# sleveque/control

Measured on AMD Instinct MI355X. Metric: Krylov iterations/s (preconditioned GMRES(10), all-at-once heat-control KKT), higher is better.
Workload: dtype f64; 1 GPU; 2-D heat control, 256^2 P1, n_t=64, beta=0.0001, T=2, BE, mode G; unknowns=8454272, krylov=gmres, left preconditioning, restart 10, classical Gram-Schmidt, parallelism=time-block rows over 1 GPU(s), transport=none, sweep_tiles=boxes from the dof coordinates (kkt_set_tile_coordinates)

## Files before the change

control_amd/csrc/tile_kernels.hip:

```cpp
#include "kernels.hpp"

#include <hip/hip_runtime.h>

#include "epilogue.hpp"

#include <algorithm>
#include <type_traits>

namespace kkt {

#define KKT_GLOBAL __attribute__((address_space(1)))
typedef KKT_GLOBAL const double *gcd_p;
typedef KKT_GLOBAL double *gd_p;
typedef KKT_GLOBAL const int32_t *gci_p;
typedef KKT_GLOBAL const uint16_t *gcu16_p;
typedef KKT_GLOBAL const uint8_t *gcb_p;
typedef KKT_GLOBAL unsigned long long *gu64_p;
typedef unsigned int u32x4 __attribute__((ext_vector_type(4)));

constexpr unsigned TILE_SPIN_LIMIT = 1u << 21;

__device__ __forceinline__ void lds_barrier() {
    asm volatile("s_waitcnt lgkmcnt(0)\n\ts_barrier" ::: "memory");
}

__device__ __forceinline__ void publish(const __amdgpu_buffer_rsrc_t rs, int grow, double v,
                                        unsigned tag) {
    const unsigned long long bits = (unsigned long long)__double_as_longlong(v);
    const u32x4 g = {(unsigned)bits, tag, (unsigned)(bits >> 32), tag};
    __builtin_amdgcn_raw_buffer_store_b128(g, rs, grow * 16, 0, 16 );
}

struct LevEarly {
    const double *vals, *dinv, *bin, *upd0;
    int32_t n_upd, prev_in_lds;
};
__device__ __forceinline__ LevEarly read_early(const TileLevel *p) {
    LevEarly f;
    f.vals = p->vals;
    f.dinv = p->dinv;
    f.bin = p->bin;
    f.upd0 = p->upd_vals[0];
    f.n_upd = p->n_upd;
    f.prev_in_lds = p->prev_in_lds;
    return f;
}

template <typename P>
__device__ __forceinline__ P opaque_ptr(P p) {
    unsigned long long u = (unsigned long long)p;
    asm volatile("" : "+v"(u));
    return (P)u;
}
__device__ __forceinline__ unsigned opaque(unsigned x) {
    asm volatile("" : "+v"(x));
    return x;
}

__device__ __forceinline__ unsigned uniform(unsigned x) { return __builtin_amdgcn_readfirstlane(x); }
template <typename P>
__device__ __forceinline__ P uniform_ptr(P p) {
    const unsigned long long u = (unsigned long long)p;
    return (P)(((unsigned long long)uniform((unsigned)(u >> 32)) << 32) | uniform((unsigned)u));
}
constexpr int TILE_NO_POLL = 0x7ffffff0;

template <int W, int RPT, int TMAX, bool UPD, int HPT_ = RPT + 1, bool COARSE = false>
__global__ __launch_bounds__(TMAX) void pc_tile_sweep(
    const TileArgs A, const TileLevel *__restrict__ levels, const int32_t *__restrict__ n_all,
    const int32_t *__restrict__ grow_all, const uint16_t *__restrict__ lcol_all,
    const int32_t *__restrict__ gpos_all, const uint8_t *__restrict__ rowmask_) {
    constexpr int HPT = HPT_;
    extern __shared__ double X[];
    __shared__ int sn[TILE_DEPTH_MAX + 1];
    __shared__ int sdead;
    __shared__ unsigned long long sstat[8];
    const int T = blockDim.x, tid = threadIdx.x, tile = blockIdx.x;
    const int nkp = A.nk_pad, depth = A.depth, its = A.its;
    const int32_t *nt = n_all + (size_t)tile * (TILE_DEPTH_MAX + 1);
    const int n0 = nt[0], nk = nt[depth], nk1 = nt[depth - 1];
    if (tid <= TILE_DEPTH_MAX) sn[tid] = nt[tid];
    if (tid < 8) sstat[tid] = 0ull;
    if (tid == 0) {
        sdead = 0;
        X[nkp - 1] = 0.0;
        X[2 * (size_t)nkp - 1] = 0.0;
    }
    __shared__ int s_bail;
    if (tid == 0) {
        typedef KKT_GLOBAL unsigned long long *gu64a_p;
        const gu64a_p ctr = (gu64a_p)(A.err + 2), bail = (gu64a_p)(A.err + 4);
        const unsigned long long nt_ = gridDim.x;
        const bool skip = A.debug_drop < 0 && tile == 0;
        unsigned long long old = 0ull;
        if (!skip) old = __hip_atomic_fetch_add(ctr, 1ull, __ATOMIC_RELAXED, __HIP_MEMORY_SCOPE_AGENT);
        else old = __hip_atomic_load(ctr, __ATOMIC_RELAXED, __HIP_MEMORY_SCOPE_AGENT);
        const unsigned long long target = (old / nt_ + 1ull) * nt_;
        int bad = 0;
        unsigned long long seen = old;
        for (int spin = 0; spin < 4096; ++spin) {
            seen = __hip_atomic_load(ctr, __ATOMIC_RELAXED, __HIP_MEMORY_SCOPE_AGENT);
            if (seen >= target) break;
            if (__hip_atomic_load(bail, __ATOMIC_RELAXED, __HIP_MEMORY_SCOPE_AGENT) == target) break;
            __builtin_amdgcn_s_sleep(8);
        }
        if (seen < target) {
            __hip_atomic_store(bail, target, __ATOMIC_RELAXED, __HIP_MEMORY_SCOPE_AGENT);
            bad = 1;
        } else if (__hip_atomic_load(bail, __ATOMIC_RELAXED, __HIP_MEMORY_SCOPE_AGENT) == target) {
            bad = 1;
        }
        if (bad) {
            atomicOr(A.err, 8u);
            if (atomicCAS(A.err + 1, 0u, 1u) == 0u) {
                A.err[17] = (unsigned)(seen - (target - nt_));
                A.err[18] = (unsigned)nt_;
            }
        }
        s_bail = bad;
    }
    __syncthreads();
    if (s_bail) return;

    const gci_p grow = (gci_p)grow_all + (size_t)tile * nkp;
    const gcb_p rowmask = (gcb_p)rowmask_;

    constexpr bool PACK = W > 9;
    constexpr int CH = PACK ? 5 : W;
    constexpr int WP = (W + 1) / 2;
    constexpr int CW = PACK ? WP : W, GW = PACK ? 1 : W;
    unsigned cpk[RPT][CW];
    int gpr[RPT][GW];
    int gr[RPT];
    bool msk[RPT];
    const gcu16_p lcol = (gcu16_p)lcol_all + (size_t)tile * RPT * W * T + tid;
    const gci_p gpos = (gci_p)gpos_all + (size_t)tile * RPT * W * T + tid;
    const gci_p gpos_base = gpos;
#pragma unroll
    for (int sl = 0; sl < RPT; ++sl) {
        const int r = sl * T + tid;
        if constexpr (PACK) {
#pragma unroll
            for (int k = 0; k < W; k += 2) {
                const unsigned lo = lcol[(size_t)(sl * W + k) * T];
                const unsigned hi = k + 1 < W ? lcol[(size_t)(sl * W + k + 1) * T] : 0u;
                cpk[sl][k / 2] = lo | (hi << 16);
            }
            gpr[sl][0] = 0;
        } else {
#pragma unroll
            for (int k = 0; k < W; ++k) {
                cpk[sl][k] = lcol[(size_t)(sl * W + k) * T];
                gpr[sl][k] = gpos[(size_t)(sl * W + k) * T];
            }
        }
        gr[sl] = r < nk1 ? grow[r] : -1;
        msk[sl] = gr[sl] >= 0 && rowmask != nullptr && rowmask[gr[sl]] != 0;
    }
    constexpr bool OPQ = PACK && TMAX > 512;
    constexpr bool TIGHT = COARSE;
    auto idx = [](const int i) { return TIGHT ? (int)opaque((unsigned)i) : i; };
    auto at = [&](const gcd_p p, const int i, const bool live) -> double {
        return live ? p[idx(i)] : 0.0;
    };
#define KKT_CPK(sl, j) (OPQ ? opaque(cpk[sl][j]) : cpk[sl][j])
#define KKT_COL(sl, k)                                                                       \
    (int)(PACK ? (((k) & 1) ? (KKT_CPK(sl, PACK ? (k) / 2 : 0) >> 16)                         \
                            : (KKT_CPK(sl, PACK ? (k) / 2 : 0) & 0xffffu))                    \
               : cpk[sl][PACK ? 0 : (k)])
#define KKT_GP(sl, k) (PACK ? gpos[(size_t)((sl) * W + (k)) * T] : gpr[sl][PACK ? 0 : (k)])
    int hl[HPT], hg[HPT];
#pragma unroll
    for (int h = 0; h < HPT; ++h) {
        const int l = n0 + h * T + tid;
        hl[h] = l < nk ? l : -1;
        hg[h] = l < nk ? grow[l] : 0;
    }

    double *scoef = X + 2 * (size_t)nkp;
    double *dump = scoef + 3 * (size_t)(COARSE ? (its > 0 ? its : 1) : (its > 1 ? its - 1 : 1));
    double *SL = dump + 1, *RC = nullptr, *EC = nullptr;
    int c_nc = 0, c_jmax = 0, c_pstride = 0, c_nslots = 0, c_nj = 0, c_slot0 = 0;
    bool c_rings = false;
    int c_njp = 0, c_jx = 0;
    unsigned cepoch = A.cepoch0;
    void *cg0 = nullptr, *cg1 = nullptr, *eg0 = nullptr, *eg1 = nullptr;
    int cg_bytes = 0, eg_bytes = 0;
    if constexpr (COARSE) {
        const TileCoarseDev *cd = A.coarse;
        cg0 = uniform_ptr((void *)cd->cg[0]);
        cg1 = uniform_ptr((void *)cd->cg[1]);
        eg0 = uniform_ptr((void *)cd->eg[0]);
        eg1 = uniform_ptr((void *)cd->eg[1]);
        cg_bytes = (int)uniform(cd->cg_bytes);
        eg_bytes = (int)uniform(cd->eg_bytes);
        c_nc = cd->nc;
        c_jmax = cd->jmax;
        c_pstride = cd->pstride;
        c_nslots = cd->nslots;
        c_nj = cd->nj[tile];
        c_slot0 = cd->slot0[tile];
        c_rings = cd->ring_prolong != 0;
        c_njp = c_rings ? cd->njx[tile] : c_nj;
        c_jx = c_rings ? cd->jxmax : c_jmax;
        RC = SL + c_nslots;
        EC = RC + c_nc;
    }
    double *RWc = nullptr, *PWc = nullptr;
    int *CSLc = nullptr, *CIPc = nullptr, *RIPc = nullptr, *JGc = nullptr;
    int *PIPc = nullptr;
    uint16_t *RROWc = nullptr, *PKc = nullptr;
    gci_p c_pip = nullptr;
    bool c_cached = true;
    int c_re0 = 0, c_pq0 = 0;
    double *EINVc = nullptr;
    bool c_einv_cache = false;
    const void *einv_key = nullptr;
    const int c_nown = COARSE ? (c_nc > tile ? (c_nc - tile + (int)gridDim.x - 1) / (int)gridDim.x : 0) : 0;
    int c_lo0 = 0, c_hi0 = 0, c_ew = 0;
    if constexpr (COARSE) {
        const TileCoarseDev *cd = A.coarse;
        c_ew = cd->ew;
        if ((int)(threadIdx.x >> 6) < c_nown) {
            const int j0 = tile + (int)(threadIdx.x >> 6) * (int)gridDim.x;
            c_lo0 = cd->e_lo[j0];
            c_hi0 = cd->e_hi[j0];
        }
        c_cached = cd->cache_lists != 0;
        const int nrm = c_cached ? cd->nr_max : 0;
        const int npm = c_rings ? cd->np_max : nrm;
        RWc = EC + c_jx;
        PWc = RWc + nrm;
        CSLc = reinterpret_cast<int *>(PWc + npm);
        CIPc = CSLc + c_nslots;
        RIPc = CIPc + (c_nc + 1);
        JGc = RIPc + (c_jmax + 1);
        PIPc = JGc + c_jx;
        RROWc = reinterpret_cast<uint16_t *>(PIPc + (c_rings ? nkp + 1 : 0));
        PKc = RROWc + nrm;
        c_einv_cache = cd->cache_einv != 0;
        EINVc = reinterpret_cast<double *>(
            (reinterpret_cast<uintptr_t>(PKc + npm) + 7) & ~(uintptr_t)7);
        const gci_p rip = (gci_p)cd->r_ip + (size_t)tile * c_jmax;
        const gci_p pip = (gci_p)cd->p_ip + (size_t)tile * c_pstride;
        const int re0 = (int)uniform((unsigned)rip[0]), re1 = (int)uniform((unsigned)rip[c_nj]);
        const int pq0 = (int)uniform((unsigned)pip[0]);
        const int pq1 = (int)uniform((unsigned)pip[c_rings ? nk : nt[0]]);
        c_re0 = re0;
        c_pq0 = pq0;
        const gcu16_p rrow = (gcu16_p)cd->r_row, pk = (gcu16_p)cd->p_k;
        const gcd_p rw = (gcd_p)cd->r_w, pw = (gcd_p)cd->p_w;
        if (c_cached) {
            for (int i = tid; i < re1 - re0; i += T) {
                RWc[i] = rw[re0 + i];
                RROWc[i] = rrow[re0 + i];
            }
            for (int i = tid; i < pq1 - pq0; i += T) {
                PWc[i] = pw[pq0 + i];
                PKc[i] = pk[pq0 + i];
            }
        }
        const gci_p cslot = (gci_p)cd->c_slot, cip = (gci_p)cd->c_ip;
        for (int i = tid; i < c_nslots; i += T) CSLc[i] = cslot[i];
        for (int i = tid; i <= c_nc; i += T) CIPc[i] = cip[i];
        const gci_p jg = (gci_p)cd->jglob + (size_t)tile * cd->jxmax;
        for (int i = tid; i <= c_nj; i += T) RIPc[i] = rip[i] - re0;
        for (int i = tid; i < c_njp; i += T) JGc[i] = jg[i];
        if (c_rings)
            for (int i = tid; i <= nk; i += T) PIPc[i] = pip[i] - pq0;
        c_pip = pip;
        __syncthreads();
    }
    const void *coef_key = nullptr;
    int cur = 0;
    unsigned epoch = A.epoch0;
    bool dead = false;
    const void *vals_key = nullptr;
    double v[RPT][W];

    unsigned long long *stat = reinterpret_cast<unsigned long long *>(A.err + 64) + (size_t)tile * 8;
    const bool stamps = A.stamps != 0;
    unsigned long long t_mark = stamps ? wall_clock64() : 0ull;
    auto lap = [&](int slot, unsigned long long count) {
        if (!stamps) return;
        const unsigned long long now = wall_clock64();
#ifndef KKT_XSTAMPS
        if (tid == 0) {
            sstat[slot] += now - t_mark;
            sstat[slot + 3] += count;
        }
#else
        if (tid == 0 && slot == 0) sstat[3] += count;
#endif
        t_mark = now;
    };

    static_assert(sizeof(TileLevel) == 128, "two scalar-cache lines per level");
    LevEarly Nf{};
    bool nf_valid = false;
    const TileLevel *nf_want = nullptr;
    auto handoff = [&](const bool both, const bool early = false) {
        lap(1, 0);
        if (nf_want != nullptr) {
            Nf = read_early(nf_want);
            nf_want = nullptr;
            nf_valid = true;
        }
        ++epoch;
        double *Xc = X + cur * nkp, *Xo = X + (cur ^ 1) * nkp;
        const __amdgpu_buffer_rsrc_t rn = __builtin_amdgcn_make_buffer_rsrc(
            uniform_ptr((void *)A.gnew[epoch & 1]), 0, (int)A.granule_bytes, 0x00020000);
        const __amdgpu_buffer_rsrc_t ro = __builtin_amdgcn_make_buffer_rsrc(
            uniform_ptr((void *)A.gold[epoch & 1]), 0, (int)A.granule_bytes, 0x00020000);
#pragma unroll
        for (int sl = 0; sl < RPT; ++sl) {
            const int r = sl * T + tid;
            if (r < n0 && !(tile == 0 && A.debug_drop > 0 && (int)(epoch - A.epoch0) == A.debug_drop)) {
                if (!early) publish(rn, gr[sl], Xc[r], epoch);
                if (both && depth > 1) publish(ro, gr[sl], Xo[r], epoch);
            }
        }
        bool want_o[HPT], need_n[HPT], need_o[HPT];
#pragma unroll
        for (int h = 0; h < HPT; ++h) {
            want_o[h] = both && hl[h] >= 0 && hl[h] < nk1;
            need_n[h] = hl[h] >= 0;
            need_o[h] = want_o[h];
        }
        auto value = [](const u32x4 g) {
            return __longlong_as_double((long long)((unsigned long long)g.x | ((unsigned long long)g.z << 32)));
        };
        for (int i = 0; i < A.poll_delay; ++i) __builtin_amdgcn_s_sleep(1);
        unsigned spins = 0;
        while (true) {
            asm volatile("" ::: "memory");
            bool ok = true;
            u32x4 tn[HPT], to[HPT];
#pragma unroll
            for (int h = 0; h < HPT; ++h) {
                tn[h] = __builtin_amdgcn_raw_buffer_load_b128(
                    rn, need_n[h] ? hg[h] * 16 : TILE_NO_POLL, 0, 16 );
                to[h] = __builtin_amdgcn_raw_buffer_load_b128(
                    ro, need_o[h] ? hg[h] * 16 : TILE_NO_POLL, 0, 16 );
            }
            __builtin_amdgcn_sched_barrier(0);
            unsigned seen[HPT][4];
#pragma unroll
            for (int h = 0; h < HPT; ++h) {
                seen[h][0] = need_n[h] ? tn[h].y : (hl[h] >= 0 ? epoch : 0u);
                seen[h][1] = need_n[h] ? tn[h].w : (hl[h] >= 0 ? epoch : 0u);
                seen[h][2] = need_o[h] ? to[h].y : (want_o[h] ? epoch : 0u);
                seen[h][3] = need_o[h] ? to[h].w : (want_o[h] ? epoch : 0u);
                const bool hit_n = need_n[h] && tn[h].y == epoch && tn[h].w == epoch;
                const bool hit_o = need_o[h] && to[h].y == epoch && to[h].w == epoch;
                if (hit_n) Xc[hl[h]] = value(tn[h]);
                if (hit_o) Xo[hl[h]] = value(to[h]);
                need_n[h] = need_n[h] && !hit_n;
                need_o[h] = need_o[h] && !hit_o;
                ok &= !need_n[h] && !need_o[h];
            }
            if (ok || dead) break;
            if (++spins >= TILE_SPIN_LIMIT) {
                dead = true;
                sdead = 1;
                atomicOr(A.err, 4u);
                if (atomicCAS(A.err + 1, 0u, 1u) == 0u) {
#pragma unroll
                    for (int h = 0; h < HPT; ++h)
                        if (need_n[h] || need_o[h]) {
                            A.err[8] = (unsigned)tile;
                            A.err[9] = epoch;
                            A.err[10] = (unsigned)hl[h];
                            A.err[11] = (unsigned)hg[h];
                            A.err[12] = seen[h][0];
                            A.err[13] = seen[h][1];
                            A.err[14] = seen[h][2];
                            A.err[15] = seen[h][3];
                            A.err[16] = both ? 1u : 0u;
                        }
                }
                break;
            }
            __builtin_amdgcn_s_sleep(1);
        }
        lds_barrier();
        dead = sdead != 0;
#ifndef KKT_XSTAMPS
        if (stamps && tid == 0) sstat[6] += spins;
#endif
        lap(0, 1);
    };

    double dinv[RPT], b[RPT];
    auto load_vals = [&](const double *ptr, const bool update_matrix) {
        vals_key = uniform_ptr((const void *)ptr);
        const gcd_p vp = (gcd_p)ptr;
        if constexpr (PACK) {
            const gci_p gpos = opaque_ptr(gpos_base);
            constexpr int G = RPT * W > 30 ? 1 : RPT;
#pragma unroll
            for (int s0 = 0; s0 < RPT; s0 += G) {
                int gp[G][W];
#pragma unroll
                for (int q = 0; q < G; ++q)
#pragma unroll
                    for (int k = 0; k < W; ++k) gp[q][k] = KKT_GP(s0 + q, k);
                __builtin_amdgcn_sched_barrier(0);
#pragma unroll
                for (int q = 0; q < G; ++q)
#pragma unroll
                    for (int k = 0; k < W; ++k)
                        v[s0 + q][k] = at(vp, gp[q][k],
                                          gp[q][k] >= 0 && (!update_matrix || gr[s0 + q] >= 0));
                __builtin_amdgcn_sched_barrier(0);
            }
        } else {
#pragma unroll
            for (int sl = 0; sl < RPT; ++sl)
#pragma unroll
                for (int k = 0; k < W; ++k) {
                    const int gp = idx(KKT_GP(sl, k));
                    v[sl][k] = at(vp, gp, gp >= 0 && (!update_matrix || idx(gr[sl]) >= 0));
                }
        }
    };
    auto load_db = [&](const LevEarly &L) {
        const gcd_p dp = (gcd_p)L.dinv, bp = (gcd_p)L.bin;
#pragma unroll
        for (int sl = 0; sl < RPT; ++sl) {
            dinv[sl] = at(dp, gr[sl], idx(gr[sl]) >= 0);
            b[sl] = at(bp, gr[sl], idx(gr[sl]) >= 0);
        }
    };
    auto load_level = [&](const LevEarly &L) {
        if (uniform_ptr((const void *)L.vals) != vals_key) load_vals(L.vals, false);
        load_db(L);
    };
    constexpr bool SEQ = (PACK || COARSE) && UPD;
    bool v_is_u = false;
    if (A.nlevels > 0) {
        const LevEarly L0 = read_early(&levels[0]);
        if (SEQ && L0.n_upd > 0) {
            load_vals(L0.upd0, true);
            load_db(L0);
            v_is_u = true;
        } else {
            load_level(L0);
        }
    }

    constexpr bool PRE = UPD && !COARSE && W * RPT <= 14 && TMAX <= 512;
    constexpr bool PRE_U = UPD && !COARSE && !PRE && W * RPT <= 7;
    constexpr int PR = PRE ? RPT : 1, PW = PRE ? W : 1;
    constexpr int UR = (PRE || PRE_U) ? RPT : 1, UW = (PRE || PRE_U) ? W : 1;
    double vn[PR][PW], un[UR][UW], dn[PR], bn[PR];
    bool pre_v = false, pre_u = false, pre_issued = false, un_loaded = false;
    auto load_un = [&](const LevEarly &N) {
        if constexpr (PRE || PRE_U) {
            pre_u = N.n_upd > 0;
            if (pre_u) {
                const gcd_p up = (gcd_p)N.upd0;
#pragma unroll
                for (int sl = 0; sl < RPT; ++sl)
#pragma unroll
                    for (int k = 0; k < W; ++k) {
                        const int gp = KKT_GP(sl, k);
                        un[sl][k] = (gr[sl] >= 0 && gp >= 0) ? up[gp] : 0.0;
                    }
            }
            un_loaded = true;
        }
    };
    auto prefetch_level = [&](const LevEarly &N) {
        if constexpr (PRE) {
            pre_issued = true;
            pre_v = uniform_ptr((const void *)N.vals) != vals_key;
            if (pre_v) {
                const gcd_p vp = (gcd_p)N.vals;
#pragma unroll
                for (int sl = 0; sl < RPT; ++sl)
#pragma unroll
                    for (int k = 0; k < W; ++k) {
                        const int gp = KKT_GP(sl, k);
                        vn[sl][k] = gp >= 0 ? vp[gp] : 0.0;
                    }
            }
            load_un(N);
            const gcd_p dp = (gcd_p)N.dinv, bp = (gcd_p)N.bin;
#pragma unroll
            for (int sl = 0; sl < RPT; ++sl) {
                dn[sl] = gr[sl] >= 0 ? dp[gr[sl]] : 0.0;
                bn[sl] = gr[sl] >= 0 ? bp[gr[sl]] : 0.0;
            }
        }
    };
    auto adopt_level = [&](const LevEarly &N) {
        if constexpr (PRE) {
            if (pre_v) {
                vals_key = uniform_ptr((const void *)N.vals);
#pragma unroll
                for (int sl = 0; sl < RPT; ++sl)
#pragma unroll
                    for (int k = 0; k < W; ++k) v[sl][k] = vn[sl][k];
            }
#pragma unroll
            for (int sl = 0; sl < RPT; ++sl) {
                dinv[sl] = dn[sl];
                b[sl] = bn[sl];
            }
        }
    };

    for (int lev = 0; lev < A.nlevels; ++lev) {
        const TileLevel &L = levels[lev];
        nf_valid = false;
        nf_want = lev + 1 < A.nlevels ? &levels[lev + 1] : nullptr;
        const bool have_u = (PRE || PRE_U) && un_loaded && pre_u;
        const bool use_v = SEQ && v_is_u;
        pre_issued = false;
        un_loaded = false;
        v_is_u = false;
        const double *einv_lev = nullptr;
        if constexpr (COARSE) {
            typedef const double *einv_entry;
            typedef __attribute__((address_space(4))) const einv_entry *einv_table_p;
            einv_lev = ((einv_table_p)(uintptr_t)A.einv)[lev];
        }
        if (uniform_ptr((const void *)L.coef) != coef_key) {
            coef_key = uniform_ptr((const void *)L.coef);
            const gcd_p cp = (gcd_p)(const double *)L.coef;
            __syncthreads();
            for (int i = idx(tid); i < 3 * (COARSE ? its : its - 1); i += T) scoef[i] = cp[i];
        }
#pragma unroll
        for (int sl = 0; sl < RPT; ++sl) {
            if constexpr (!(SEQ && COARSE)) {
#pragma unroll
                for (int k = 0; k < W; ++k) asm volatile("" : "+v"(v[sl][k]));
            }
            asm volatile("" : "+v"(dinv[sl]));
            asm volatile("" : "+v"(b[sl]));
        }
        if (!COARSE && stamps && tid == 0) sstat[7] += wall_clock64() - t_mark;
        const double post1 = L.post1, post2 = L.post2;
        int cr;
        {
            double *Xc = X + cur * nkp, *Xo = X + (cur ^ 1) * nkp;
            if (UPD && L.n_upd > 0) {
                if (!L.prev_in_lds) {
                    const gcd_p xp = (gcd_p)L.x_prev;
                    for (int l = idx(tid); l < nk; l += T) Xc[l] = xp[grow[l]];
                    lds_barrier();
                }
                double acc[RPT];
#pragma unroll
                for (int sl = 0; sl < RPT; ++sl) acc[sl] = 0.0;
                if constexpr (PRE || PRE_U) {
                    if (have_u) {
                        double xu[UR][UW];
#pragma unroll
                        for (int sl = 0; sl < RPT; ++sl)
#pragma unroll
                            for (int k = 0; k < W; ++k) xu[sl][k] = Xc[KKT_COL(sl, k)];
                        __builtin_amdgcn_sched_barrier(0);
#pragma unroll
                        for (int k = 0; k < W; ++k)
#pragma unroll
                            for (int sl = 0; sl < RPT; ++sl)
                                acc[sl] = __builtin_fma(un[sl][k], xu[sl][k], acc[sl]);
                    }
                }
                if constexpr (SEQ) {
                    if (use_v) {
#pragma unroll
                        for (int sl = 0; sl < RPT; ++sl) {
                            if (sl * T + (tid & ~63) >= nk1) continue;
#pragma unroll
                            for (int k0 = 0; k0 < W; k0 += CH) {
                                double xv[CH];
#pragma unroll
                                for (int k = 0; k < CH; ++k)
                                    if (k0 + k < W) xv[k] = Xc[KKT_COL(sl, k0 + k)];
#pragma unroll
                                for (int k = 0; k < CH; ++k)
                                    if (k0 + k < W)
                                        acc[sl] = __builtin_fma(v[sl][k0 + k], xv[k], acc[sl]);
                                __builtin_amdgcn_sched_barrier(0);
                            }
                        }
                    }
                }
                if constexpr (!(PACK && SEQ))
                for (int t = (have_u || use_v) ? 1 : 0; t < L.n_upd; ++t) {
                    const gcd_p up = (gcd_p)L.upd_vals[t];
#pragma unroll
                    for (int sl = 0; sl < RPT; ++sl) {
                        if (sl * T + (tid & ~63) >= nk1) continue;
#pragma unroll
                        for (int k0 = 0; k0 < W; k0 += CH) {
                            int gp[CH];
                            double vu[CH];
#pragma unroll
                            for (int k = 0; k < CH; ++k)
                                if (k0 + k < W) gp[k] = idx(KKT_GP(sl, k0 + k));
#pragma unroll
                            for (int k = 0; k < CH; ++k)
                                if (k0 + k < W)
                                    vu[k] = at(up, gp[k], idx(gr[sl]) >= 0 && gp[k] >= 0);
#pragma unroll
                            for (int k = 0; k < CH; ++k)
                                if (k0 + k < W)
                                    acc[sl] = __builtin_fma(vu[k], Xc[KKT_COL(sl, k0 + k)], acc[sl]);
                            if constexpr (PACK) __builtin_amdgcn_sched_barrier(0);
                        }
                    }
                }
                if constexpr (SEQ && COARSE) {
                    if (uniform_ptr((const void *)L.vals) != vals_key) load_vals(L.vals, false);
                }
                const gd_p bo = (gd_p)L.bout;
#pragma unroll
                for (int sl = 0; sl < RPT; ++sl) {
                    const int r = sl * T + tid;
                    const double out =
                        msk[sl] ? 0.0 : epi_lin(L.ca, acc[sl], true, L.cy, b[sl], false, 0.0, 0.0);
                    const double out2 = epi_first(L.p1_scale, dinv[sl], out);
                    b[sl] = out;
                    if (r < nk1) Xo[r] = out2;
                    if (r < n0 && bo != nullptr) bo[idx(gr[sl])] = out;
                }
                if constexpr (SEQ && !COARSE) {
                    if (uniform_ptr((const void *)L.vals) != vals_key) load_vals(L.vals, false);
                }
            } else {
                const bool last = its == 1;
                const double q1 = last ? post1 : 1.0, q2 = last ? post2 : 1.0;
#pragma unroll
                for (int sl = 0; sl < RPT; ++sl) {
                    const int r = sl * T + tid;
                    double out = 0.0;
                    if (!msk[sl])
                        out = epi_cheb(false, 0.0, 0.0, false, 0.0, 0.0, L.p1_scale, dinv[sl], b[sl],
                                       0.0, q1, q2);
                    if (r < nk1) Xo[r] = out;
                }
            }
            cr = depth - 1;
            lds_barrier();
            cur ^= 1;
        }
        const bool has_next = lev + 1 < A.nlevels;
        if (PRE && has_next && its - 1 <= cr) {
            Nf = read_early(&levels[lev + 1]);
            nf_want = nullptr;
            nf_valid = true;
            prefetch_level(Nf);
        }
#pragma unroll
        for (int sl = 0; sl < RPT; ++sl) {
            if constexpr (SEQ && !COARSE) {
#pragma unroll
                for (int k = 0; k < W; ++k) asm volatile("" : "+v"(v[sl][k]));
            }
            asm volatile("" : "+v"(dinv[sl]));
            asm volatile("" : "+v"(b[sl]));
        }
        lap(2, 1);
        if constexpr (COARSE) {
            auto cstep = [&](const int mode, const int nv, const double cf1, const double cf2,
                             const double cf3, const bool has_old, const double q1,
                             const double q2) {
                double *Xc = X + cur * nkp, *Xo = X + (cur ^ 1) * nkp;
#pragma unroll
                for (int sl = 0; sl < RPT; ++sl) {
                    if (sl * T + (tid & ~63) >= nv) continue;
                    const int r = sl * T + tid;
                    double acc = 0.0;
#pragma unroll
                    for (int k0 = 0; k0 < W; k0 += CH) {
                        double xv[CH];
#pragma unroll
                        for (int k = 0; k < CH; ++k)
                            if (k0 + k < W) xv[k] = Xc[KKT_COL(sl, k0 + k)];
#pragma unroll
                        for (int k = 0; k < CH; ++k)
                            if (k0 + k < W) acc = __builtin_fma(v[sl][k0 + k], xv[k], acc);
                        if constexpr (PACK) __builtin_amdgcn_sched_barrier(0);
                    }
                    if (r < nv) {
                        double out = 0.0;
                        if (!msk[sl]) {
                            if (mode == 0) {
                                out = epi_cheb(has_old, cf1, Xo[r], true, cf2, Xc[r], cf3, dinv[sl],
                                               b[sl], acc, q1, q2);
                            } else {
                                out = b[sl] - acc;
                            }
                        }
                        Xo[r] = out;
                    }
                }
            };
            const TileCoarseDev *cd = A.coarse;
            const gcd_p einv = (gcd_p)einv_lev;
            const int wave = tid >> 6, lane = tid & 63, nwaves = T >> 6;
            for (int cyc = 0; cyc < A.cycles; ++cyc) {
                if (cyc == 0) {
                    double *Xo = X + (cur ^ 1) * nkp;
#pragma unroll
                    for (int sl = 0; sl < RPT; ++sl) {
                        const int r = sl * T + tid;
                        if (r < n0) Xo[r] = b[sl];
                    }
                } else {
                    if (cr == 0 || (c_rings && cr < depth)) {
                        handoff(false);
                        cr = depth;
                    }
                    cstep(1, n0, 0.0, 0.0, 0.0, false, 1.0, 1.0);
                }
                lds_barrier();
                lap(1, cyc == 0 ? 0 : 1);
#ifdef KKT_XSTAMPS
                unsigned long long xs_t = wall_clock64();
                auto xs = [&](int slot) {
                    const unsigned long long n_ = wall_clock64();
                    if (tid == 0) sstat[slot] += n_ - xs_t;
                    xs_t = n_;
                };
#define KKT_XS(slot) xs(slot)
#else
#define KKT_XS(slot)
#endif
                ++cepoch;
                {
                    int pe0[RPT], pe1[RPT];
                    if (!c_rings) {
#pragma unroll
                        for (int sl = 0; sl < RPT; ++sl) {
                            const int r = sl * T + tid;
                            pe0[sl] = r < n0 ? c_pip[r] - c_pq0 : 0;
                            pe1[sl] = r < n0 ? c_pip[r + 1] - c_pq0 : 0;
                        }
                    }
                    const double *Rb = X + (cur ^ 1) * nkp;
                    const __amdgpu_buffer_rsrc_t rc_ = __builtin_amdgcn_make_buffer_rsrc(
                        (cepoch & 1) ? cg1 : cg0, 0, cg_bytes, 0x00020000);
                    for (int k = wave; k < c_nj; k += nwaves) {
                        const int e0 = RIPc[k], e1 = RIPc[k + 1];
                        double a = 0.0;
                        if (c_cached) {
                            for (int e = e0 + lane; e < e1; e += 64)
                                a = __builtin_fma(RWc[e], Rb[RROWc[e]], a);
                        } else {
                            const gcu16_p rrow = (gcu16_p)cd->r_row + c_re0;
                            const gcd_p rw = (gcd_p)cd->r_w + c_re0;
                            for (int e = e0 + lane; e < e1; e += 64)
                                a = __builtin_fma(rw[e], Rb[rrow[e]], a);
                        }
#pragma unroll
                        for (int o = 32; o > 0; o >>= 1) a += __shfl_xor(a, o, 64);
                        if (lane == 0) publish(rc_, c_slot0 + k, a, cepoch);
                    }
                    constexpr int CSL = 4;
                    KKT_XS(0);
                    for (int i = 0; i < A.poll_delay; ++i) __builtin_amdgcn_s_sleep(1);
                    for (int base = 0; base < c_nslots; base += CSL * T) {
                        bool need[CSL];
#pragma unroll
                        for (int q = 0; q < CSL; ++q) need[q] = base + q * T + tid < c_nslots;
                        const bool live0 = need[0];
                        unsigned spins = 0;
                        while (true) {
                            asm volatile("" ::: "memory");
                            bool ok = true;
                            u32x4 t[CSL];
#pragma unroll
                            for (int q = 0; q < CSL; ++q)
                                t[q] = __builtin_amdgcn_raw_buffer_load_b128(
                                    rc_, need[q] ? (base + q * T + tid) * 16 : TILE_NO_POLL, 0, 16);
                            __builtin_amdgcn_sched_barrier(0);
                            const unsigned seen_y = need[0] ? t[0].y : (live0 ? cepoch : 0u);
                            const unsigned seen_w = need[0] ? t[0].w : (live0 ? cepoch : 0u);
#pragma unroll
                            for (int q = 0; q < CSL; ++q) {
                                const bool hit = need[q] && t[q].y == cepoch && t[q].w == cepoch;
                                if (hit)
                                    SL[base + q * T + tid] = __longlong_as_double((long long)(
                                        (unsigned long long)t[q].x | ((unsigned long long)t[q].z << 32)));
                                need[q] = need[q] && !hit;
                                ok &= !need[q];
                            }
                            if (ok || dead) break;
                            if (++spins >= TILE_SPIN_LIMIT) {
                                dead = true;
                                sdead = 1;
                                atomicOr(A.err, 4u);
                                if (atomicCAS(A.err + 1, 0u, 1u) == 0u) {
                                    A.err[8] = (unsigned)tile;
                                    A.err[9] = cepoch;
                                    A.err[10] = 0xffffu;
                                    A.err[11] = (unsigned)(base + tid);
                                    A.err[12] = seen_y;
                                    A.err[13] = seen_w;
                                    A.err[16] = 2u;
                                }
                                break;
                            }
                            __builtin_amdgcn_s_sleep(1);
                        }
                    }
                    KKT_XS(1);
                    lds_barrier();
                    KKT_XS(2);
                    dead = sdead != 0;
                    for (int j = tid; j < c_nc; j += T) {
                        double a = 0.0;
                        for (int q = CIPc[j]; q < CIPc[j + 1]; ++q) a += SL[CSLc[q]];
                        RC[j] = a;
                    }
                    lds_barrier();
                    KKT_XS(4);
                    const __amdgpu_buffer_rsrc_t re_ = __builtin_amdgcn_make_buffer_rsrc(
                        (cepoch & 1) ? eg1 : eg0, 0, eg_bytes, 0x00020000);
                    const int ntl = (int)gridDim.x;
                    const gci_p elo = (gci_p)cd->e_lo, ehi = (gci_p)cd->e_hi;
                    if (c_einv_cache && uniform_ptr((const void *)einv) != einv_key) {
                        for (int i = wave; i < c_nown; i += nwaves) {
                            const int j = tile + i * ntl;
                            const int lo = i == wave ? c_lo0 : elo[j], hi = i == wave ? c_hi0 : ehi[j];
                            const gcd_p row = einv + (size_t)j * c_nc;
                            for (int q = lo + lane; q < hi; q += 64)
                                EINVc[(size_t)i * c_ew + (q - lo)] = row[q];
                        }
                        einv_key = uniform_ptr((const void *)einv);
                    }
                    for (int i = wave; i < c_nown; i += nwaves) {
                        double a = 0.0;
                        const int j = tile + i * ntl;
                        const int lo = i == wave ? c_lo0 : elo[j], hi = i == wave ? c_hi0 : ehi[j];
                        if (c_einv_cache) {
                            const double *row = EINVc + (size_t)i * c_ew;
                            for (int q = lo + lane; q < hi; q += 64)
                                a = __builtin_fma(row[q - lo], RC[q], a);
                        } else {
                            const gcd_p row = einv + (size_t)j * c_nc;
                            constexpr int EU = 8;
                            for (int q0 = lo + lane; q0 < hi; q0 += 64 * EU) {
                                double rv[EU];
#pragma unroll
                                for (int u = 0; u < EU; ++u) {
                                    const int q = q0 + 64 * u;
                                    rv[u] = q < hi ? row[q] : 0.0;
                                }
#pragma unroll
                                for (int u = 0; u < EU; ++u) {
                                    const int q = q0 + 64 * u;
                                    if (q < hi) a = __builtin_fma(rv[u], RC[q], a);
                                }
                            }
                        }
#pragma unroll
                        for (int o = 32; o > 0; o >>= 1) a += __shfl_xor(a, o, 64);
                        if (lane == 0) publish(re_, tile + i * ntl, a, cepoch);
                    }
                    KKT_XS(5);
                    for (int k0 = 0; k0 < c_njp; k0 += T) {
                        const int k = k0 + tid;
                        u32x4 g = u32x4{0u, 0u, 0u, 0u};
                        unsigned spins = 0;
                        while (true) {
                            asm volatile("" ::: "memory");
                            bool ok = true;
                            if (k < c_njp && (g.y != cepoch || g.w != cepoch)) {
                                g = __builtin_amdgcn_raw_buffer_load_b128(re_, JGc[k] * 16, 0, 16);
                                ok = g.y == cepoch && g.w == cepoch;
                            }
                            if (__all(ok) || dead) break;
                            if (++spins >= TILE_SPIN_LIMIT) {
                                dead = true;
                                sdead = 1;
                                atomicOr(A.err, 4u);
                                if (atomicCAS(A.err + 1, 0u, 1u) == 0u) {
                                    A.err[8] = (unsigned)tile;
                                    A.err[9] = cepoch;
                                    A.err[10] = 0xfffeu;
                                    A.err[11] = (unsigned)(k < c_njp ? JGc[k] : 0);
                                    A.err[12] = g.y;
                                    A.err[13] = g.w;
                                    A.err[16] = 2u;
                                }
                                break;
                            }
                            __builtin_amdgcn_s_sleep(1);
                        }
                        if (k < c_njp)
                            EC[k] = __longlong_as_double((long long)(
                                (unsigned long long)g.x | ((unsigned long long)g.z << 32)));
                    }
                    lds_barrier();
                    dead = sdead != 0;
                    KKT_XS(6);
                    double *Xc = X + cur * nkp;
                    if (c_rings) {
                        for (int l = tid; l < nk; l += T) {
                            double a = 0.0;
                            for (int e = PIPc[l]; e < PIPc[l + 1]; ++e)
                                a = __builtin_fma(PWc[e], EC[PKc[e]], a);
                            Xc[l] = cyc == 0 ? a : Xc[l] + a;
                        }
                    } else {
#pragma unroll
                    for (int sl = 0; sl < RPT; ++sl) {
                        const int r = sl * T + tid;
                        if (r < n0) {
                            double a = 0.0;
                            if (c_cached) {
                                for (int e = pe0[sl]; e < pe1[sl]; ++e)
                                    a = __builtin_fma(PWc[e], EC[PKc[e]], a);
                            } else {
                                const gcu16_p pk = (gcu16_p)cd->p_k + c_pq0;
                                const gcd_p pw = (gcd_p)cd->p_w + c_pq0;
                                for (int e = pe0[sl]; e < pe1[sl]; ++e)
                                    a = __builtin_fma(pw[e], EC[pk[e]], a);
                            }
                            Xc[r] = cyc == 0 ? a : Xc[r] + a;
                        }
                    }
                    }
                }
                int nv_next = sn[depth - 1];
                double cn1 = scoef[0], cn2 = scoef[1], cn3 = scoef[2];
#pragma unroll
                for (int sl = 0; sl < RPT; ++sl)
#pragma unroll
                    for (int k = 0; k < W; ++k) asm volatile("" : "+v"(v[sl][k]));
                lds_barrier();
                if (stamps) {
                    const unsigned long long now = wall_clock64();
                    if (tid == 0) sstat[7] += now - t_mark;
                    t_mark = now;
                }
                if (!c_rings) handoff(false);
                cr = depth;
                for (int s = 1; s <= its; ++s) {
                    if (cr == 0) {
                        handoff(s >= 2);
                        cr = depth;
                    }
                    const bool last = cyc + 1 == A.cycles && s == its;
                    cstep(0, nv_next, cn1, cn2, cn3, s >= 2, last ? post1 : 1.0, last ? post2 : 1.0);
                    if (s < its) {
                        nv_next = sn[(cr - 1 == 0 ? depth : cr - 1) - 1];
                        cn1 = scoef[3 * s];
                        cn2 = scoef[3 * s + 1];
                        cn3 = scoef[3 * s + 2];
                    }
                    lds_barrier();
                    cur ^= 1;
                    --cr;
                }
            }
        } else {
            int nv_next = sn[(cr == 0 ? depth : cr) - 1];
            double cn1 = scoef[0], cn2 = scoef[1], cn3 = scoef[2];
            bool early_done = false;
            for (int s = 2; s <= its; ++s) {
                if (cr == 0) {
                    handoff(s >= 3, early_done);
                    early_done = false;
                    cr = depth;
                    if (PRE && has_next && its - s < depth) prefetch_level(Nf);
                }
                const int nv = nv_next;
                const double cf1 = cn1, cf2 = cn2, cf3 = cn3;
                const bool last = s == its;
                const double q1 = last ? post1 : 1.0, q2 = last ? post2 : 1.0;
                const bool has_old = s >= 3;
                double *Xc = X + cur * nkp, *Xo = X + (cur ^ 1) * nkp;
                const bool pub_next = PACK && cr == 1 && s < its;
                const bool pub_drop =
                    tile == 0 && A.debug_drop > 0 && (int)(epoch + 1 - A.epoch0) == A.debug_drop;
                early_done = pub_next;
                const __amdgpu_buffer_rsrc_t rn_next = __builtin_amdgcn_make_buffer_rsrc(
                    (void *)A.gnew[(epoch + 1) & 1], 0, (int)A.granule_bytes, 0x00020000);
                if constexpr (PACK) {
    #pragma unroll
                    for (int sl = 0; sl < RPT; ++sl) {
                        if (sl * T + (tid & ~63) >= nv) continue;
                        const int r = sl * T + tid;
                        double acc = 0.0;
    #pragma unroll
                        for (int k0 = 0; k0 < W; k0 += CH) {
                            double xv[CH];
    #pragma unroll
                            for (int k = 0; k < CH; ++k)
                                if (k0 + k < W) xv[k] = Xc[KKT_COL(sl, k0 + k)];
    #pragma unroll
                            for (int k = 0; k < CH; ++k)
                                if (k0 + k < W) acc = __builtin_fma(v[sl][k0 + k], xv[k], acc);
                            __builtin_amdgcn_sched_barrier(0);
                        }
                        if (r < nv) {
                            const double e0 = Xo[r], e1 = Xc[r];
                            double out = 0.0;
                            if (!msk[sl])
                                out = epi_cheb(has_old, cf1, e0, true, cf2, e1, cf3, dinv[sl], b[sl],
                                               acc, q1, q2);
                            Xo[r] = out;
                            if (pub_next && !pub_drop && r < n0)
                                publish(rn_next, gr[sl], out, epoch + 1);
                        }
                    }
                } else {
                    int nl = 0;
                    long long keep[RPT];
    #pragma unroll
                    for (int sl = 0; sl < RPT; ++sl) {
                        if (sl * T + (tid & ~63) < nv) nl = sl + 1;
                        keep[sl] = msk[sl] ? 0ll : -1ll;
                        asm volatile("" : "+v"(keep[sl]));
                    }
                    auto body = [&](auto NLc) {
                        constexpr int NL = decltype(NLc)::value;
                        double xv[NL][W], e0[NL], e1[NL], acc[NL];
    #pragma unroll
                        for (int sl = 0; sl < NL; ++sl) {
    #pragma unroll
                            for (int k = 0; k < W; ++k) xv[sl][k] = Xc[KKT_COL(sl, k)];
                            const int r = sl * T + tid;
                            e0[sl] = Xo[r];
                            e1[sl] = Xc[r];
                            acc[sl] = 0.0;
                        }
                        __builtin_amdgcn_sched_barrier(0);
    #pragma unroll
                        for (int k = 0; k < W; ++k)
    #pragma unroll
                            for (int sl = 0; sl < NL; ++sl)
                                acc[sl] = __builtin_fma(v[sl][k], xv[sl][k], acc[sl]);
    #pragma unroll
                        for (int sl = 0; sl < NL; ++sl) {
                            const int r = sl * T + tid;
                            double t = has_old ? cf1 * e0[sl] : 0.0;
                            t += cf2 * e1[sl];
                            t += cf3 * (dinv[sl] * (b[sl] - acc[sl]));
                            const double out = __longlong_as_double(
                                __double_as_longlong(q2 * (q1 * t)) & keep[sl]);
                            *(r < nv ? Xo + r : dump) = out;
                        }
                    };
                    if (nl == 1) body(std::integral_constant<int, 1>{});
                    if constexpr (RPT >= 2)
                        if (nl == 2) body(std::integral_constant<int, 2>{});
                    if constexpr (RPT >= 3)
                        if (nl == 3) body(std::integral_constant<int, 3>{});
                }
                if (s < its) {
                    const int crn = cr - 1 == 0 ? depth : cr - 1;
                    nv_next = sn[crn - 1];
                    cn1 = scoef[3 * (s - 1)];
                    cn2 = scoef[3 * (s - 1) + 1];
                    cn3 = scoef[3 * (s - 1) + 2];
                }
                lds_barrier();
                cur ^= 1;
                --cr;
            }
        }
        lap(1, (unsigned long long)(its - 1));
        if constexpr (SEQ && COARSE) {
#pragma unroll
            for (int sl = 0; sl < RPT; ++sl)
#pragma unroll
                for (int k = 0; k < W; ++k) asm volatile("" : "+v"(v[sl][k]));
        }
        {
            double *Xc = X + cur * nkp;
            const gd_p op = (gd_p)L.out;
#pragma unroll
            for (int sl = 0; sl < RPT; ++sl) {
                const int r = sl * T + tid;
                if (r < n0) op[idx(gr[sl])] = Xc[r];
            }
            if (lev + 1 < A.nlevels) {
                if (!nf_valid) Nf = read_early(&levels[lev + 1]);
                nf_want = nullptr;
                const LevEarly &N = Nf;
                if constexpr (SEQ && COARSE) {
                    const bool upd = N.n_upd > 0 &&
                                     (PACK || uniform_ptr((const void *)N.vals) != vals_key);
                    const double *src = upd ? N.upd0 : N.vals;
                    if (upd || uniform_ptr((const void *)src) != vals_key) load_vals(src, upd);
                    load_db(N);
                    v_is_u = upd;
                } else if (!(PRE && pre_issued)) {
                    if (SEQ && N.n_upd > 0) {
                        load_vals(N.upd0, true);
                        load_db(N);
                        v_is_u = true;
                    } else {
                        load_level(N);
                        if constexpr (PRE_U) load_un(N);
                    }
                }
                if (N.n_upd > 0 && N.prev_in_lds) handoff(false);
                if (PRE && pre_issued) adopt_level(N);
            }
        }
    }
    if (stamps && tid == 0)
        for (int i = 0; i < 8; ++i) stat[i] += sstat[i];
}

#undef KKT_COL
#undef KKT_CPK
#undef KKT_GP

typedef void (*tile_fn)(const TileArgs, const TileLevel *, const int32_t *, const int32_t *,
                        const uint16_t *, const int32_t *, const uint8_t *);
static tile_fn pick_tile_coarse(int W, int rpt, int threads, int hslots);
static tile_fn pick_tile(int W, int rpt, int threads, bool fused = true, int hslots = 0,
                         bool coarse = false) {
    if (coarse) return fused ? pick_tile_coarse(W, rpt, threads, hslots) : nullptr;
    if (hslots <= 0) hslots = 1;
#define KKT_T(w)                                                           \
    if (W == w) {                                                          \
        if (threads <= 512) {                                              \
            switch (rpt) {                                                 \
                case 1: return pc_tile_sweep<w, 1, 512, true>;             \
                case 2: return pc_tile_sweep<w, 2, 512, true>;             \
                case 3: return pc_tile_sweep<w, 3, 512, true>;             \
                default: return nullptr;                                   \
            }                                                              \
        }                                                                  \
        return rpt == 1 ? pc_tile_sweep<w, 1, 1024, true> : nullptr;       \
    }
    KKT_T(5) KKT_T(7) KKT_T(9)
#undef KKT_T
    if (W == 15 && threads > 512 && rpt == 1 && hslots <= 1)
        return fused ? pc_tile_sweep<15, 1, 1024, true, 1> : pc_tile_sweep<15, 1, 1024, false, 1>;
    if (W == 15 && threads <= 512) {
        if (rpt == 1) return fused ? pc_tile_sweep<15, 1, 512, true> : pc_tile_sweep<15, 1, 512, false>;
        if (rpt == 2) return fused ? pc_tile_sweep<15, 2, 512, true> : pc_tile_sweep<15, 2, 512, false>;
    }
    if (W == 19 && threads <= 512 && rpt == 1)
        return fused ? pc_tile_sweep<19, 1, 512, true> : pc_tile_sweep<19, 1, 512, false>;
    if (W == 19 && threads <= 512 && rpt == 2)
        return fused ? pc_tile_sweep<19, 2, 512, true> : pc_tile_sweep<19, 2, 512, false>;
    if (W == 19 && threads > 512 && threads <= 768 && rpt == 1)
        return fused ? pc_tile_sweep<19, 1, 768, true> : pc_tile_sweep<19, 1, 768, false>;
    return nullptr;
}

static tile_fn pick_tile_coarse(int W, int rpt, int threads, int hslots) {
    if (hslots <= 0) hslots = 1;
#define KKT_TC(w)                                                                  \
    if (W == w) {                                                                  \
        if (threads <= 512) {                                                      \
            switch (rpt) {                                                         \
                case 1: return pc_tile_sweep<w, 1, 512, true, 2, true>;            \
                case 2: return pc_tile_sweep<w, 2, 512, true, 3, true>;            \
                case 3: return pc_tile_sweep<w, 3, 512, true, 4, true>;            \
                default: return nullptr;                                           \
            }                                                                      \
        }                                                                          \
        return rpt == 1 ? pc_tile_sweep<w, 1, 1024, true, 2, true> : nullptr;      \
    }
    KKT_TC(5) KKT_TC(7) KKT_TC(9)
#undef KKT_TC
    if (W == 15 && threads > 512 && rpt == 1 && hslots <= 1)
        return pc_tile_sweep<15, 1, 1024, true, 1, true>;
    if (W == 15 && threads <= 512) {
        if (rpt == 1) return pc_tile_sweep<15, 1, 512, true, 2, true>;
        if (rpt == 2) return pc_tile_sweep<15, 2, 512, true, 3, true>;
    }
    if (W == 19 && threads <= 512 && rpt == 1) return pc_tile_sweep<19, 1, 512, true, 2, true>;
    if (W == 19 && threads <= 512 && rpt == 2) return pc_tile_sweep<19, 2, 512, true, 3, true>;
    if (W == 19 && threads > 512 && threads <= 768 && rpt == 1)
        return pc_tile_sweep<19, 1, 768, true, 2, true>;
    return nullptr;
}

bool tile_sweep_coarse_available(int W, int rpt, int threads, int hslots) {
    return threads >= 64 && threads <= 1024 && threads % 64 == 0 && hslots <= rpt + 1 &&
           pick_tile_coarse(W, rpt, threads, hslots) != nullptr;
}

bool tile_sweep_fuses_update(int W, int max_terms) {
    return W <= 9 || ((W == 15 || W == 19) && max_terms <= 1);
}

size_t tile_sweep_lds_bytes(int nk_pad, int its, int coarse_nc, int coarse_nslots, int coarse_jmax,
                            int coarse_nr_max, int coarse_einv_rows, int coarse_einv_width,
                            int coarse_ring_entries, int coarse_jxmax) {
    if (coarse_nc > 0 && coarse_einv_rows > 0)
        return tile_sweep_lds_bytes(nk_pad, its, coarse_nc, coarse_nslots, coarse_jmax,
                                    coarse_nr_max, 0, 0, coarse_ring_entries, coarse_jxmax) +
               (size_t)coarse_einv_rows * (coarse_einv_width > 0 ? coarse_einv_width : coarse_nc) *
                   sizeof(double) + 8;
    if (coarse_nc > 0) {
        const bool rings = coarse_jxmax > 0;
        const size_t jx = rings ? (size_t)coarse_jxmax : (size_t)coarse_jmax;
        const size_t np = (size_t)coarse_nr_max + (rings ? (size_t)coarse_ring_entries : 0);
        const size_t pip = rings ? (size_t)nk_pad + 1 : 0;
        return (2 * (size_t)nk_pad + 3 * (size_t)std::max(1, its) + 1 + (size_t)coarse_nslots +
                (size_t)coarse_nc + jx + (size_t)coarse_nr_max + np) * sizeof(double) +
               ((size_t)coarse_nslots + (size_t)coarse_nc + 1 + (size_t)coarse_jmax + 1 + jx + pip) *
                   sizeof(int) +
               ((size_t)coarse_nr_max + np) * sizeof(uint16_t) + 16;
    }
    return (2 * (size_t)nk_pad + 3 * (size_t)std::max(1, its - 1) + 1) * sizeof(double);
}

size_t tile_sweep_lds_bytes(int nk_pad, int its, const TileCoarseDev &c, int cache, bool rings) {
    const bool r = rings && cache >= 1;
    return tile_sweep_lds_bytes(nk_pad, its, c.nc, c.nslots, c.jmax, cache >= 1 ? c.nr_max : 0,
                                cache == 2 ? c.nown : 0, c.ew, r ? c.np_max - c.nr_max : 0,
                                r ? c.jxmax : 0);
}

size_t tile_sweep_lds_bytes(int nk_pad, int its, const TileCoarseDev &c) {
    return tile_sweep_lds_bytes(nk_pad, its, c, c.cache_einv ? 2 : c.cache_lists ? 1 : 0,
                                c.ring_prolong != 0);
}

int tile_sweep_max_rpt(int W, int threads) {
    int best = 0;
    for (int rpt = 1; rpt <= 4; ++rpt)
        if (pick_tile(W, rpt, threads, true, 1)) best = rpt;
    return best;
}

int tile_sweep_max_hslots(int W, int rpt, int threads) {
    int best = 0;
    for (int h = 1; h <= rpt + 1; ++h)
        if (pick_tile(W, rpt, threads, true, h)) best = h;
    return best;
}

bool tile_sweep_available(int W, int rpt, int threads, int hslots) {
    return threads >= 64 && threads <= 1024 && threads % 64 == 0 && hslots <= rpt + 1 &&
           pick_tile(W, rpt, threads, true, hslots) != nullptr;
}

int tile_sweep_max_tiles(int W, int rpt, int threads, size_t lds_bytes, int hslots, bool coarse) {
    int dev = 0, cus = 0;
    if (hipGetDevice(&dev) != hipSuccess) return 0;
    if (hipDeviceGetAttribute(&cus, hipDeviceAttributeMultiprocessorCount, dev) != hipSuccess) return 0;
    for (int fused = coarse ? 1 : 0; fused < 2; ++fused) {
        tile_fn f = pick_tile(W, rpt, threads, fused != 0, hslots, coarse);
        int per_cu = 0;
        if (!f) return 0;
        if (lds_bytes > 48 * 1024 &&
            hipFuncSetAttribute((const void *)f, hipFuncAttributeMaxDynamicSharedMemorySize,
                                (int)lds_bytes) != hipSuccess)
            return 0;
        if (hipOccupancyMaxActiveBlocksPerMultiprocessor(&per_cu, f, threads, lds_bytes) != hipSuccess)
            return 0;
        if (per_cu < 1) return 0;
    }
    return cus;
}

void launch_tile_sweep(hipStream_t s, const TileArgs &a, const TileLevel *d_levels,
                       const int32_t *d_n, const int32_t *d_grow, const uint16_t *d_lcol,
                       const int32_t *d_gpos, const uint8_t *d_rowmask, int ntiles, int threads,
                       size_t granule_words, const TileCoarseDev *h_coarse) {
    if (a.nlevels <= 0 || ntiles <= 0) return;
    auto chk = [](hipError_t e, const char *what) {
        if (e != hipSuccess)
            throw TileLaunchError{std::string("tile sweep program: ") + what + ": " +
                                  hipGetErrorString(e)};
    };
    (void)hipGetLastError();
    if (a.clear) {
        if (a.clear & 1)
            for (int i = 0; i < 2; ++i) {
                launch_zero_bytes(s, a.gnew[i], granule_words * sizeof(unsigned long long));
                launch_zero_bytes(s, a.gold[i], granule_words * sizeof(unsigned long long));
            }
        if (h_coarse && (a.clear & 2))
            for (int i = 0; i < 2; ++i) {
                launch_zero_bytes(s, h_coarse->cg[i], h_coarse->cg_bytes);
                launch_zero_bytes(s, h_coarse->eg[i], h_coarse->eg_bytes);
            }
        chk(hipGetLastError(), "clearing the granule buffers");
    }
    const size_t lds = h_coarse ? tile_sweep_lds_bytes(a.nk_pad, a.its, *h_coarse)
                                : tile_sweep_lds_bytes(a.nk_pad, a.its);
    tile_fn f = pick_tile(a.W, a.rpt, threads, a.fused_update != 0, a.hslots, h_coarse != nullptr);
    if (!f) throw TileLaunchError{"tile sweep program: no kernel variant for this plan"};
    (void)hipGetLastError();
    hipLaunchKernelGGL(f, dim3(ntiles), dim3(threads), lds, s, a, d_levels, d_n, d_grow, d_lcol,
                       d_gpos, d_rowmask);
    chk(hipGetLastError(), "launch");
}

}
```

Baseline: 162.8 Krylov iterations/s.

## Use permlane/DPP wave reductions and batch LDS gathers in coarse correction

Replaces the shuffle-based wave reductions with a permlane32/permlane16 swap plus DPP row-shift sequence that leaves the sum in lane 0. Batches the LDS gathers in the coarse restriction sum, the cached E^-1 row dot product, and the prolongation rows, so several independent loads are issued before they are consumed. The intent is to shorten LDS latency chains in the coarse-grid correction phase. It also rewrites the EINV pointer alignment in terms of X and changes the XSTAMPS instrumentation. These touch several unrelated spots and add register pressure.

Result: faster. 169.7 Krylov iterations/s, median of 6 (+4.2%).

```diff
diff --git a/control_amd/csrc/tile_kernels.hip b/control_amd/csrc/tile_kernels.hip
--- a/control_amd/csrc/tile_kernels.hip
+++ b/control_amd/csrc/tile_kernels.hip
@@ -64,6 +64,65 @@
     return (P)(((unsigned long long)uniform((unsigned)(u >> 32)) << 32) | uniform((unsigned)u));
 }
 constexpr int TILE_NO_POLL = 0x7ffffff0;
+
+
+__device__ __forceinline__ double wave_sum_lane0(double a) {
+    auto halves = [](const double x, unsigned &lo, unsigned &hi) {
+        const unsigned long long b = (unsigned long long)__double_as_longlong(x);
+        lo = (unsigned)b;
+        hi = (unsigned)(b >> 32);
+    };
+    auto whole = [](const unsigned lo, const unsigned hi) {
+        return __longlong_as_double((long long)((unsigned long long)lo | ((unsigned long long)hi << 32)));
+    };
+    unsigned lo, hi;
+    halves(a, lo, hi);
+    {
+        const auto l = __builtin_amdgcn_permlane32_swap(lo, lo, false, false);
+        const auto h = __builtin_amdgcn_permlane32_swap(hi, hi, false, false);
+        a = whole(l[0], h[0]) + whole(l[1], h[1]);
+    }
+    halves(a, lo, hi);
+    {
+        const auto l = __builtin_amdgcn_permlane16_swap(lo, lo, false, false);
+        const auto h = __builtin_amdgcn_permlane16_swap(hi, hi, false, false);
+        a = whole(l[0], h[0]) + whole(l[1], h[1]);
+    }
+#define KKT_ROW_SHL(n)                                                                          \
+    {                                                                                           \
+        halves(a, lo, hi);                                                                      \
+        const unsigned l = (unsigned)__builtin_amdgcn_update_dpp(0, (int)lo, 0x100 + (n), 0xf, 0xf, true); \
+        const unsigned h = (unsigned)__builtin_amdgcn_update_dpp(0, (int)hi, 0x100 + (n), 0xf, 0xf, true); \
+        a += whole(l, h);                                                                       \
+    }
+    KKT_ROW_SHL(8)
+    KKT_ROW_SHL(4)
+    KKT_ROW_SHL(2)
+    KKT_ROW_SHL(1)
+#undef KKT_ROW_SHL
+    return a;
+}
+
+template <int U>
+__device__ __forceinline__ double prolong_row(const int e0, const int e1, const uint16_t *pk,
+                                              const double *pw, const double *ec) {
+    int k[U];
+    double w[U], x[U];
+#pragma unroll
+    for (int u = 0; u < U; ++u) {
+        const int e = e0 + u < e1 ? e0 + u : 0;
+        k[u] = pk[e];
+        w[u] = pw[e];
+    }
+#pragma unroll
+    for (int u = 0; u < U; ++u) x[u] = ec[k[u]];
+    double a = 0.0;
+#pragma unroll
+    for (int u = 0; u < U; ++u)
+        if (e0 + u < e1) a = __builtin_fma(w[u], x[u], a);
+    for (int e = e0 + U; e < e1; ++e) a = __builtin_fma(pw[e], ec[pk[e]], a);
+    return a;
+}
 
 template <int W, int RPT, int TMAX, bool UPD, int HPT_ = RPT + 1, bool COARSE = false>
 __global__ __launch_bounds__(TMAX) void pc_tile_sweep(
@@ -239,8 +298,8 @@
         RROWc = reinterpret_cast<uint16_t *>(PIPc + (c_rings ? nkp + 1 : 0));
         PKc = RROWc + nrm;
         c_einv_cache = cd->cache_einv != 0;
-        EINVc = reinterpret_cast<double *>(
-            (reinterpret_cast<uintptr_t>(PKc + npm) + 7) & ~(uintptr_t)7);
+        EINVc = X + (static_cast<size_t>(reinterpret_cast<const char *>(PKc + npm) -
+                                         reinterpret_cast<const char *>(X)) + 7) / 8;
         const gci_p rip = (gci_p)cd->r_ip + (size_t)tile * c_jmax;
         const gci_p pip = (gci_p)cd->p_ip + (size_t)tile * c_pstride;
         const int re0 = (int)uniform((unsigned)rip[0]), re1 = (int)uniform((unsigned)rip[c_nj]);
@@ -290,7 +349,8 @@
             sstat[slot + 3] += count;
         }
 #else
-        if (tid == 0 && slot == 0) sstat[3] += count;
+        (void)slot;
+        (void)count;
 #endif
         t_mark = now;
     };
@@ -758,8 +818,7 @@
                             for (int e = e0 + lane; e < e1; e += 64)
                                 a = __builtin_fma(rw[e], Rb[rrow[e]], a);
                         }
-#pragma unroll
-                        for (int o = 32; o > 0; o >>= 1) a += __shfl_xor(a, o, 64);
+                        a = wave_sum_lane0(a);
                         if (lane == 0) publish(rc_, c_slot0 + k, a, cepoch);
                     }
                     constexpr int CSL = 4;
@@ -814,9 +873,21 @@
                     lds_barrier();
                     KKT_XS(2);
                     dead = sdead != 0;
+                    constexpr int CU = 4;
                     for (int j = tid; j < c_nc; j += T) {
+                        const int q0 = CIPc[j], q1 = CIPc[j + 1];
+                        int cs[CU];
+                        double cp[CU];
+#pragma unroll
+                        for (int k = 0; k < CU; ++k) cs[k] = CSLc[q0 + k < q1 ? q0 + k : 0];
+#pragma unroll
+                        for (int k = 0; k < CU; ++k) cp[k] = SL[cs[k]];
+                        asm volatile("" : "+v"(cp[0]));
                         double a = 0.0;
-                        for (int q = CIPc[j]; q < CIPc[j + 1]; ++q) a += SL[CSLc[q]];
+#pragma unroll
+                        for (int k = 0; k < CU; ++k)
+                            if (q0 + k < q1) a += cp[k];
+                        for (int q = q0 + CU; q < q1; ++q) a += SL[CSLc[q]];
                         RC[j] = a;
                     }
                     lds_barrier();
@@ -840,9 +911,20 @@
                         const int j = tile + i * ntl;
                         const int lo = i == wave ? c_lo0 : elo[j], hi = i == wave ? c_hi0 : ehi[j];
                         if (c_einv_cache) {
+                            constexpr int EG = 6;
                             const double *row = EINVc + (size_t)i * c_ew;
-                            for (int q = lo + lane; q < hi; q += 64)
-                                a = __builtin_fma(row[q - lo], RC[q], a);
+                            for (int qb = lo + lane; qb < hi; qb += 64 * EG) {
+                                double rv[EG], xc[EG];
+#pragma unroll
+                                for (int u = 0; u < EG; ++u) {
+                                    const int q = qb + 64 * u < hi ? qb + 64 * u : qb;
+                                    rv[u] = row[q - lo];
+                                    xc[u] = RC[q];
+                                }
+#pragma unroll
+                                for (int u = 0; u < EG; ++u)
+                                    if (qb + 64 * u < hi) a = __builtin_fma(rv[u], xc[u], a);
+                            }
                         } else {
                             const gcd_p row = einv + (size_t)j * c_nc;
                             constexpr int EU = 8;
@@ -860,8 +942,7 @@
                                 }
                             }
                         }
-#pragma unroll
-                        for (int o = 32; o > 0; o >>= 1) a += __shfl_xor(a, o, 64);
+                        a = wave_sum_lane0(a);
                         if (lane == 0) publish(re_, tile + i * ntl, a, cepoch);
                     }
                     KKT_XS(5);
@@ -904,10 +985,10 @@
                     double *Xc = X + cur * nkp;
                     if (c_rings) {
                         for (int l = tid; l < nk; l += T) {
-                            double a = 0.0;
-                            for (int e = PIPc[l]; e < PIPc[l + 1]; ++e)
-                                a = __builtin_fma(PWc[e], EC[PKc[e]], a);
-                            Xc[l] = cyc == 0 ? a : Xc[l] + a;
+                            const int e0 = PIPc[l], e1 = PIPc[l + 1];
+                            const double xo = Xc[l];
+                            const double a = prolong_row<4>(e0, e1, PKc, PWc, EC);
+                            Xc[l] = cyc == 0 ? a : xo + a;
                         }
                     } else {
 #pragma unroll
@@ -916,8 +997,7 @@
                         if (r < n0) {
                             double a = 0.0;
                             if (c_cached) {
-                                for (int e = pe0[sl]; e < pe1[sl]; ++e)
-                                    a = __builtin_fma(PWc[e], EC[PKc[e]], a);
+                                a = prolong_row<4>(pe0[sl], pe1[sl], PKc, PWc, EC);
                             } else {
                                 const gcu16_p pk = (gcu16_p)cd->p_k + c_pq0;
                                 const gcd_p pw = (gcd_p)cd->p_w + c_pq0;
@@ -936,6 +1016,7 @@
 #pragma unroll
                     for (int k = 0; k < W; ++k) asm volatile("" : "+v"(v[sl][k]));
                 lds_barrier();
+                KKT_XS(3);
                 if (stamps) {
                     const unsigned long long now = wall_clock64();
                     if (tid == 0) sstat[7] += now - t_mark;
```
